# Regenerator/dpf-nets

Hardware: AMD Instinct MI355X
Metric: points/sec through 14-layer flow + Chamfer, B=32 N=2048 (higher is better)
Workload: dtype f16x3 MFMA operands, fp32 accumulate/points; 1 GPU; configs[1]: airplane autoencoder shapes, B=32 N=2048 per GPU: 14 coupling layers (first 14 of LocalCondRNVPDecoder(n_flows=5)), direct/eval-BN, + nn_distance both directions + CD reduction; clouds_per_gpu=32, points_per_cloud=2048, hidden=64, latent=128, global_clouds=32, per_layer_lists=False, launch=hipGraph replay, 10 step(s) per graph, steps_in_flight=1, settle_steps=400, parallelism=clouds sharded, no collective, sclk_mhz=2239, chamfer_impl=auto (matrix-core filtered exact search at this size)

## Files before the change

### dpf_nets_amd/csrc/chamfer_mfma.hip

```cpp
#include <hip/hip_runtime.h>
#include <limits.h>
#include <stdint.h>
#include <stdlib.h>

#include "dpf_hip.h"
#include "lds_attr.h"
#include "zero_fill.h"
#include "nn_refscan.h"

#pragma clang fp contract(off)

namespace {

typedef __bf16 bf16x8 __attribute__((ext_vector_type(8)));
typedef float f32x16 __attribute__((ext_vector_type(16)));
typedef uint32_t u32x4 __attribute__((ext_vector_type(4)));

constexpr int CT = dispatch::NNM_CT;
constexpr int PROW = 100;
constexpr int SCH = 32;
constexpr int WCAP = SCH * 64 / 8;
constexpr int NNM_PTS = CT * 1024, NNM_LISTS = NNM_PTS + CT * PROW * 4;
__host__ __device__ constexpr int nnm_lds_bytes(int qw) { return NNM_LISTS + qw * SCH * 64 + qw * WCAP * 2; }

__device__ __forceinline__ uint32_t f2u(float x) { return __builtin_bit_cast(uint32_t, x); }
__device__ __forceinline__ float u2f(uint32_t x) { return __builtin_bit_cast(float, x); }
__device__ __forceinline__ uint32_t bf16_rne(float x) {
    const uint32_t u = f2u(x);
    return (u + 0x7FFFu + ((u >> 16) & 1u)) >> 16;
}
__device__ __forceinline__ void split2(float x, uint32_t &hi, uint32_t &lo) {
    const uint32_t h = f2u(x) & 0xFFFF0000u;
    hi = h >> 16;
    lo = bf16_rne(x - u2f(h));
}

__host__ __device__ inline int tiles_of(int n) { return (n + 31) / 32; }

__device__ __forceinline__ void cand_coord(float c, uint32_t &w0, uint32_t &w1) {
    uint32_t hi, lo;
    split2(c, hi, lo);
    w0 = hi | (hi << 16);
    w1 = lo | (lo << 16);
}
__device__ __forceinline__ void cand_fragment(float x, float y, float z, bool live, uint4 &h0, uint4 &h1) {
    cand_coord(x, h0.x, h0.y);
    cand_coord(y, h0.z, h0.w);
    cand_coord(z, h1.x, h1.y);
    const float w = (x * x + y * y) + z * z;
    const float ww = live ? w : 3.0e38f;
    const uint32_t wh = f2u(ww) & 0xFFFF0000u;
    const float r1 = ww - u2f(wh);
    const uint32_t wm = f2u(r1) & 0xFFFF0000u;
    const float r2 = r1 - u2f(wm);
    h1.z = (wh >> 16) | (live ? wm : 0u);
    h1.w = live ? bf16_rne(r2) : 0u;
}
__device__ __forceinline__ uint4 query_fragment(float x, float y, float z, int h) {
    uint32_t ah, al, bh, bl;
    split2(-2.0f * (h ? z : x), ah, al);
    split2(-2.0f * y, bh, bl);
    uint4 o;
    o.x = ah | (al << 16); o.y = o.x;
    o.z = h ? 0x3F803F80u : (bh | (bl << 16));
    o.w = h ? 0x00003F80u : o.z;
    return o;
}

struct MDir {
    const float *q, *c;
    float *dist;
    int *idx;
    int nq, nc;
    long qstride, cstride;
};
struct MArgs {
    MDir d[2]; int pn2; float *part; unsigned *ticket; float *cd;
#ifdef DPF_PROFILE
    unsigned long long *prof;
#endif
};

__device__ __forceinline__ f32x16 mfma(uint4 a, uint4 b) {
    const f32x16 z = {0.f, 0.f, 0.f, 0.f, 0.f, 0.f, 0.f, 0.f, 0.f, 0.f, 0.f, 0.f, 0.f, 0.f, 0.f, 0.f};
    return __builtin_amdgcn_mfma_f32_32x32x16_bf16(__builtin_bit_cast(bf16x8, a), __builtin_bit_cast(bf16x8, b), z, 0, 0, 0);
}
__device__ __forceinline__ float tile_min(const f32x16 &s) {
    float m = fminf(fminf(s[0], s[1]), s[2]);
    m = fminf(fminf(m, s[3]), s[4]);   m = fminf(fminf(m, s[5]), s[6]);
    m = fminf(fminf(m, s[7]), s[8]);   m = fminf(fminf(m, s[9]), s[10]);
    m = fminf(fminf(m, s[11]), s[12]); m = fminf(fminf(m, s[13]), s[14]);
    return fminf(fminf(m, s[15]), s[0]);
}
__device__ __forceinline__ float dist3(float cx, float cy, float cz, float qx, float qy, float qz) {
    const float dx = cx - qx, dy = cy - qy, dz = cz - qz;
    return (dx * dx + dy * dy) + dz * dz;
}
template <class P>
__device__ __forceinline__ void exact_tile(P cp, int nc, int t, int tl, int h, float qx, float qy, float qz,
                                           float &best, int &bidx) {
    float d[16];
#pragma unroll
    for (int g = 0; g < 4; ++g) {
        const float *row = cp + (size_t)tl * PROW + 8 * g + 4 * h;
        const float4 vx = *(const float4 *)row, vy = *(const float4 *)(row + 32), vz = *(const float4 *)(row + 64);
        d[4 * g + 0] = dist3(vx.x, vy.x, vz.x, qx, qy, qz); d[4 * g + 1] = dist3(vx.y, vy.y, vz.y, qx, qy, qz);
        d[4 * g + 2] = dist3(vx.z, vy.z, vz.z, qx, qy, qz); d[4 * g + 3] = dist3(vx.w, vy.w, vz.w, qx, qy, qz);
    }
    float m = fminf(fminf(d[0], d[1]), d[2]);
#pragma unroll
    for (int r = 3; r < 15; r += 2) m = fminf(fminf(m, d[r]), d[r + 1]);
    m = fminf(m, d[15]);
    if (m <= best) {
        int kmin = INT_MAX;
#pragma unroll
        for (int r = 15; r >= 0; --r) {
            const int k = t * 32 + 8 * (r >> 2) + 4 * h + (r & 3);
            kmin = (d[r] == m && k < nc) ? k : kmin;
        }
        const bool better = kmin != INT_MAX && (m < best || kmin < bidx);
        best = better ? m : best;
        bidx = better ? kmin : bidx;
    }
}

template <class P>
__device__ __forceinline__ void exact_tile_mk(P cp, int nc, int t, int tl, int h, float qx, float qy, float qz, float &m, int &kmin) {
    float d[16];
#pragma unroll
    for (int g = 0; g < 4; ++g) {
        const float *row = cp + (size_t)tl * PROW + 8 * g + 4 * h;
        const float4 vx = *(const float4 *)row, vy = *(const float4 *)(row + 32), vz = *(const float4 *)(row + 64);
        d[4 * g + 0] = dist3(vx.x, vy.x, vz.x, qx, qy, qz); d[4 * g + 1] = dist3(vx.y, vy.y, vz.y, qx, qy, qz);
        d[4 * g + 2] = dist3(vx.z, vy.z, vz.z, qx, qy, qz); d[4 * g + 3] = dist3(vx.w, vy.w, vz.w, qx, qy, qz);
    }
    m = fminf(fminf(d[0], d[1]), d[2]);
#pragma unroll
    for (int r = 3; r < 15; r += 2) m = fminf(fminf(m, d[r]), d[r + 1]);
    m = fminf(m, d[15]);
    int rmin = 16;
#pragma unroll
    for (int r = 15; r >= 0; --r) rmin = d[r] == m ? r : rmin;
    const int k = t * 32 + 8 * (rmin >> 2) + 4 * h + (rmin & 3);
    kmin = (rmin < 16 && k < nc) ? k : INT_MAX;
}

template <int CTRL, int ROW_MASK = 0xF>
__device__ __forceinline__ unsigned dpp_or0(unsigned v) {
    return (unsigned)__builtin_amdgcn_update_dpp(0, (int)v, CTRL, ROW_MASK, 0xF, true);
}
__device__ __forceinline__ unsigned wave_scan_add(unsigned v) {
    v += dpp_or0<0x111>(v); v += dpp_or0<0x112>(v); v += dpp_or0<0x114>(v); v += dpp_or0<0x118>(v);
    v += dpp_or0<0x142, 0xA>(v);
    v += dpp_or0<0x143, 0xC>(v);
    return v;
}
__device__ __forceinline__ unsigned wave_max_u32(unsigned v) {
    v = max(v, dpp_or0<0x111>(v)); v = max(v, dpp_or0<0x112>(v)); v = max(v, dpp_or0<0x114>(v)); v = max(v, dpp_or0<0x118>(v));
    v = max(v, dpp_or0<0x142, 0xA>(v));
    v = max(v, dpp_or0<0x143, 0xC>(v));
    return (unsigned)__builtin_amdgcn_readlane((int)v, 63);
}

#ifdef DPF_PROFILE
#define DPF_T(i) { __builtin_amdgcn_sched_barrier(0); \
    if (prof_at != nullptr) { const unsigned long long t_ = __builtin_amdgcn_s_memtime(); if ((threadIdx.x & 63) == 0) prof_at[i] = t_; } \
    __builtin_amdgcn_sched_barrier(0); }
#else
#define DPF_T(i)
#endif

typedef __attribute__((address_space(3))) void lds_void;
typedef __attribute__((address_space(1))) const void glb_void;

template <int QW>
__global__ __launch_bounds__(QW * 64) void nnm_kernel(MArgs args) {
    extern __shared__ __attribute__((aligned(16))) uint8_t lds[];
    unsigned char *qtile = (unsigned char *)(lds + NNM_LISTS);
    __shared__ float s_r2[QW], s_sum[QW];
    const bool pairwise = args.pn2 > 0;
    const int dir = pairwise ? (int)(blockIdx.z & 1) : (int)blockIdx.z;
    const MDir A = args.d[dir];
    const int pi = pairwise ? (int)(blockIdx.z >> 1) : 0, pj = (int)blockIdx.y;
    const int bi = pairwise ? 0 : (int)blockIdx.y;
    const int nq = A.nq, nc = A.nc;
    const bool sums = args.part != nullptr;
    const size_t part_at = pairwise ? (((size_t)pi * args.pn2 + pj) * 2 + dir) * gridDim.x + blockIdx.x
                                    : ((size_t)bi * 2 + dir) * gridDim.x + blockIdx.x;
    const size_t unit = pairwise ? (size_t)pi * args.pn2 + pj : (size_t)bi;
    auto publish = [&](float t) {
        if (args.ticket == nullptr) { args.part[part_at] = t; return; }
        __hip_atomic_store(&args.part[part_at], t, __ATOMIC_RELAXED, __HIP_MEMORY_SCOPE_AGENT);
        asm volatile("s_waitcnt vmcnt(0)" ::: "memory");
        const unsigned nwg2 = 2u * gridDim.x;
        const unsigned old = __hip_atomic_fetch_add(&args.ticket[unit], 1u, __ATOMIC_RELAXED, __HIP_MEMORY_SCOPE_AGENT);
        if (old == nwg2 - 1) {
            const float *p = args.part + unit * nwg2;
            float s1 = 0.f, s2 = 0.f;
            for (unsigned x0 = 0; x0 < gridDim.x; x0 += 4) {
                float v1[4], v2[4];
#pragma unroll
                for (unsigned u = 0; u < 4; ++u) {
                    const unsigned x = min(x0 + u, gridDim.x - 1);
                    v1[u] = __hip_atomic_load(&p[x], __ATOMIC_RELAXED, __HIP_MEMORY_SCOPE_AGENT);
                    v2[u] = __hip_atomic_load(&p[gridDim.x + x], __ATOMIC_RELAXED, __HIP_MEMORY_SCOPE_AGENT);
                }
#pragma unroll
                for (unsigned u = 0; u < 4; ++u)
                    if (x0 + u < gridDim.x) { s1 += v1[u]; s2 += v2[u]; }
            }
            args.cd[unit] = s1 / (float)args.d[0].nq + s2 / (float)args.d[1].nq;
            __hip_atomic_store(&args.ticket[unit], 0u, __ATOMIC_RELAXED, __HIP_MEMORY_SCOPE_AGENT);
        }
    };
    if ((int)blockIdx.x * QW * 32 >= nq) {
        if (sums && threadIdx.x == 0) publish(0.f);
        return;
    }
    const int tid = threadIdx.x, lane = tid & 63, h = lane >> 5;
    const int wave = __builtin_amdgcn_readfirstlane(tid >> 6);
#ifdef DPF_PROFILE
    unsigned long long *prof_at = nullptr;
    if (args.prof != nullptr && blockIdx.y < 2 && blockIdx.z == 0 && gridDim.x <= 4)
        prof_at = args.prof + ((size_t)(blockIdx.y * gridDim.x + blockIdx.x) * QW + wave) * 16;
#endif
    DPF_T(0)
    const int qt = blockIdx.x * QW + wave;
    const int nqt = tiles_of(nq), nct = tiles_of(nc);
    const bool wave_live = qt < nqt;
    const size_t qcloud = pairwise ? (size_t)(dir == 0 ? pi : pj) * A.qstride : (size_t)bi * A.qstride;
    const size_t ccloud = pairwise ? (size_t)(dir == 0 ? pj : pi) * A.cstride : (size_t)bi * A.cstride;
    const float *__restrict__ cpts = A.c + ccloud;
    const int j = qt * 32 + (lane & 31);
    const float *qsrc = A.q + qcloud + (size_t)min(j, nq - 1) * 3;
    const float qx = qsrc[0], qy = qsrc[1], qz = qsrc[2];
    constexpr int KPT = CT * 32 / (QW * 64);
    const int npass = (nct + CT - 1) / CT;
    float px[KPT], py[KPT], pz[KPT];
#pragma unroll
    for (int k = 0; k < KPT; ++k) {
        const int p = tid + k * QW * 64;
        px[k] = 0.f; py[k] = 0.f; pz[k] = 0.f;
        if (p < nc) { const float *src = cpts + (size_t)p * 3; px[k] = src[0]; py[k] = src[1]; pz[k] = src[2]; }
    }
    float mux, muy, muz;
    {
        const float *src = cpts + (size_t)min(lane, nc - 1) * 3;
        mux = src[0]; muy = src[1]; muz = src[2];
        for (int d = 32; d > 0; d >>= 1) { mux += __shfl_xor(mux, d); muy += __shfl_xor(muy, d); muz += __shfl_xor(muz, d); }
        mux *= 0.015625f; muy *= 0.015625f; muz *= 0.015625f;
    }
    const float qcx = qx - mux, qcy = qy - muy, qcz = qz - muz;
    const uint4 bq = query_fragment(qcx, qcy, qcz, h);
    const float INF_ = __builtin_inff();
    float r2 = j < nq ? (qcx * qcx + qcy * qcy) + qcz * qcz : 0.f;
    r2 = nn_not_finite(r2) ? INF_ : r2;
    DPF_T(1)
    if (nct > CT)
        for (int p = tid; p < nc; p += QW * 64) {
            const float *src = cpts + (size_t)p * 3;
            const float x = src[0] - mux, y = src[1] - muy, z = src[2] - muz;
            const float cn = (x * x + y * y) + z * z;
            r2 = nn_not_finite(cn) ? INF_ : fmaxf(r2, cn);
        }

    uint4 *sfrag = (uint4 *)lds;
    float *spts = (float *)(lds + NNM_PTS);
    auto put = [&](int pl, bool live, float x, float y, float z) {
        const int t = pl >> 5, i = pl & 31;
        uint4 f0, f1;
        const float cx = live ? x - mux : 0.f, cy = live ? y - muy : 0.f, cz = live ? z - muz : 0.f;
        cand_fragment(cx, cy, cz, live, f0, f1);
        sfrag[t * 64 + i] = f0;
        sfrag[t * 64 + 32 + i] = f1;
        spts[t * PROW + i] = live ? x : 3.0e38f; spts[t * PROW + 32 + i] = live ? y : 3.0e38f; spts[t * PROW + 64 + i] = live ? z : 3.0e38f;
        return (cx * cx + cy * cy) + cz * cz;
    };
    {
        const int tn = min(CT, nct);
        int tidp = tid;
        asm volatile("" : "+v"(tidp));
#pragma unroll
        for (int k = 0; k < KPT; ++k) {
            const int pl = tidp + k * QW * 64;
            if ((pl >> 5) < tn) {
                const float cn = put(pl, pl < nc, px[k], py[k], pz[k]);
                r2 = nn_not_finite(cn) ? INF_ : fmaxf(r2, cn);
            }
        }
    }
    DPF_T(2)
    const float r2w = u2f(wave_max_u32(f2u(r2)));
    if (lane == 0) s_r2[wave] = r2w;
    __syncthreads();
    float tau;
    bool slow;
    {
        float m = s_r2[0];
#pragma unroll
        for (int w = 1; w < QW; ++w) m = fmaxf(m, s_r2[w]);
        tau = m * 2.44140625e-4f;
        slow = nn_not_finite(m);
    }
    DPF_T(3)

    unsigned short *wl = (unsigned short *)(lds + NNM_LISTS + QW * SCH * 64) + (size_t)wave * WCAP;
    uint2 *res = (uint2 *)(qtile + (size_t)wave * SCH * 64);
    float smin = __builtin_inff();
    float best = __builtin_inff();
    int bidx = INT_MAX;
    for (int pass = 0; pass < (slow ? 0 : npass); ++pass) {
        const int t0 = pass * CT, tn = min(CT, nct - t0);
        if (pass > 0) {
            __syncthreads();
            int tidp = tid;
            asm volatile("" : "+v"(tidp));
#pragma unroll
            for (int k = 0; k < KPT; ++k) {
                const int pl = tidp + k * QW * 64, p = t0 * 32 + pl;
                if ((pl >> 5) < tn) {
                    const bool live = p < nc;
                    float x = 0.f, y = 0.f, z = 0.f;
                    if (live) { const float *src = cpts + (size_t)p * 3; x = src[0]; y = src[1]; z = src[2]; }
                    put(pl, live, x, y, z);
                }
            }
            __syncthreads();
        }
        if (wave_live) {
            for (int c0 = 0; c0 < tn; c0 += SCH) {
                const int cn = min(SCH, tn - c0);
                float mt[SCH];
                if (cn == SCH) {
                    const uint4 *fr = sfrag + c0 * 64 + lane;
                    if constexpr (QW < 16) {
                        uint4 fa = fr[0], fb = fr[64];
                        f32x16 a = mfma(fa, bq);
                        fa = fr[2 * 64];
#pragma unroll
                        for (int u = 0; u < SCH; u += 2) {
                            const f32x16 b = mfma(fb, bq);
                            if (u + 3 < SCH) fb = fr[(u + 3) * 64];
                            __builtin_amdgcn_sched_barrier(0);
                            mt[u] = tile_min(a);
                            __builtin_amdgcn_sched_barrier(0);
                            if (u + 2 < SCH) {
                                a = mfma(fa, bq);
                                if (u + 4 < SCH) fa = fr[(u + 4) * 64];
                            }
                            __builtin_amdgcn_sched_barrier(0);
                            mt[u + 1] = tile_min(b);
                            __builtin_amdgcn_sched_barrier(0);
                        }
                    } else {
                        f32x16 a = mfma(fr[0], bq);
#pragma unroll
                        for (int u = 0; u < SCH; u += 2) {
                            const f32x16 b = mfma(fr[(u + 1) * 64], bq);
                            __builtin_amdgcn_sched_barrier(0);
                            mt[u] = tile_min(a);
                            __builtin_amdgcn_sched_barrier(0);
                            if (u + 2 < SCH) a = mfma(fr[(u + 2) * 64], bq);
                            __builtin_amdgcn_sched_barrier(0);
                            mt[u + 1] = tile_min(b);
                            __builtin_amdgcn_sched_barrier(0);
                        }
                    }
                } else {
                    auto frag = [&](int u) { return sfrag[(c0 + min(u, cn - 1)) * 64 + lane]; };
                    f32x16 a = mfma(frag(0), bq);
#pragma unroll
                    for (int u = 0; u < SCH; u += 2) {
                        const f32x16 b = mfma(frag(u + 1), bq);
                        __builtin_amdgcn_sched_barrier(0);
                        mt[u] = tile_min(a);
                        __builtin_amdgcn_sched_barrier(0);
                        if (u + 2 < SCH) a = mfma(frag(u + 2), bq);
                        __builtin_amdgcn_sched_barrier(0);
                        mt[u + 1] = tile_min(b);
                        __builtin_amdgcn_sched_barrier(0);
                    }
                }
                DPF_T(4 + 5 * (c0 / SCH))
                float cm = fminf(fminf(mt[0], mt[1]), mt[2]);
#pragma unroll
                for (int u = 3; u + 1 < SCH; u += 2) cm = fminf(fminf(cm, mt[u]), mt[u + 1]);
                cm = fminf(cm, mt[SCH - 1]);
                smin = fminf(smin, cm);
                const float thr = fminf(smin, __shfl_xor(smin, 32)) + tau;
                unsigned smask = 0;
                static_assert(SCH == 32, "the mask is built sixteen tiles at a time, twice");
#define NNM_MK(n) "v_cmp_le_f32 vcc, %" #n ", %17\n\tv_addc_co_u32 %0, vcc, %0, %0, vcc\n\t"
#pragma unroll
                for (int u = 0; u < SCH; u += 16)
                    asm(NNM_MK(1) NNM_MK(2) NNM_MK(3) NNM_MK(4) NNM_MK(5) NNM_MK(6) NNM_MK(7) NNM_MK(8)
                        NNM_MK(9) NNM_MK(10) NNM_MK(11) NNM_MK(12) NNM_MK(13) NNM_MK(14) NNM_MK(15) NNM_MK(16)
                        : "+v"(smask)
                        : "v"(mt[u]), "v"(mt[u + 1]), "v"(mt[u + 2]), "v"(mt[u + 3]), "v"(mt[u + 4]), "v"(mt[u + 5]), "v"(mt[u + 6]),
                          "v"(mt[u + 7]), "v"(mt[u + 8]), "v"(mt[u + 9]), "v"(mt[u + 10]), "v"(mt[u + 11]), "v"(mt[u + 12]),
                          "v"(mt[u + 13]), "v"(mt[u + 14]), "v"(mt[u + 15]), "v"(thr)
                        : "vcc");
#undef NNM_MK
                if (cn < SCH) smask &= ~0u << (SCH - cn);
                const int nsurv = __builtin_popcount(smask);
                DPF_T(5 + 5 * (c0 / SCH))
                int off = (int)wave_scan_add((unsigned)nsurv);
                const int W = __builtin_amdgcn_readlane(off, 63);
                off -= nsurv;
                if (W <= WCAP) {
                    {
                        unsigned mk = smask;
                        for (int e = 0; __builtin_amdgcn_ballot_w64(mk != 0) != 0; ++e) {
                            if (mk != 0) wl[off + e] = (unsigned short)((lane << 8) | (SCH - 1 - __builtin_ctz(mk)));
                            mk &= mk - 1;
                        }
                    }
                    DPF_T(6 + 5 * (c0 / SCH))
                    __builtin_amdgcn_fence(__ATOMIC_RELEASE, "wavefront");
                    __builtin_amdgcn_wave_barrier();
                    for (int i0 = 0; i0 < W; i0 += 64) {
                        const int i = i0 + lane;
                        const unsigned item = wl[min(i, W - 1)];
                        const int sl = (int)(item >> 8), tl = c0 + (int)(item & 255u);
                        const float sx = __shfl(qx, sl), sy = __shfl(qy, sl), sz = __shfl(qz, sl);
                        float m; int k;
                        exact_tile_mk(spts, nc, t0 + tl, tl, sl >> 5, sx, sy, sz, m, k);
                        if (i < W) res[i] = make_uint2(__float_as_uint(m), (unsigned)k);
                    }
                    __builtin_amdgcn_fence(__ATOMIC_RELEASE, "wavefront");
                    __builtin_amdgcn_wave_barrier();
                    DPF_T(7 + 5 * (c0 / SCH))
                    for (int e = 0; __builtin_amdgcn_ballot_w64(e < nsurv) != 0; ++e) {
                        if (e < nsurv) {
                            const uint2 r = res[off + e];
                            const float m = __uint_as_float(r.x);
                            const int k = (int)r.y;
                            const bool better = k != INT_MAX && (m < best || (m == best && k < bidx));
                            best = better ? m : best;
                            bidx = better ? k : bidx;
                        }
                    }
                    __builtin_amdgcn_fence(__ATOMIC_RELEASE, "wavefront");
                    __builtin_amdgcn_wave_barrier();
                    DPF_T(8 + 5 * (c0 / SCH))
                } else {
                    const int smax = (int)wave_max_u32((unsigned)nsurv);
                    unsigned mk = smask;
                    for (int e = 0; e < smax; ++e) {
                        const bool take = mk != 0;
                        const int tl = c0 + (take ? SCH - 1 - __builtin_ctz(mk) : 0);
                        mk &= mk - 1;
                        float b2 = best; int i2 = bidx;
                        exact_tile(spts, nc, t0 + tl, tl, h, qx, qy, qz, b2, i2);
                        if (take) { best = b2; bidx = i2; }
                    }
                }
            }
        }
    }
    if (slow && wave_live)
        nn_reference_scan(cpts, nc, qx, qy, qz, best, bidx);
    if (!wave_live && !sums) return;
    const float od = __shfl_xor(best, 32);
    const int oi = __shfl_xor(bidx, 32);
    if (od < best || (od == best && oi < bidx)) { best = od; bidx = oi; }
    int tid_out = threadIdx.x;
    asm volatile("" : "+v"(tid_out));
    const int j_out = (blockIdx.x * QW + (tid_out >> 6)) * 32 + (tid_out & 31);
    if (!pairwise) {
        if (wave_live && h == 0 && j_out < nq) {
            A.dist[(size_t)bi * nq + j_out] = best;
            A.idx[(size_t)bi * nq + j_out] = bidx;
        }
        if (!sums) return;
    }
    DPF_T(14)
    float sum = (wave_live && h == 0 && j_out < nq) ? best : 0.f;
    for (int d = 16; d > 0; d >>= 1) sum += __shfl_xor(sum, d);
    if (lane == 0) s_sum[wave] = sum;
    __syncthreads();
    if (tid == 0) {
        float t = s_sum[0];
#pragma unroll
        for (int w = 1; w < QW; ++w) t += s_sum[w];
        publish(t);
    }
    DPF_T(15)
}

__global__ __launch_bounds__(64) void nnm_surrogate_kernel(const float *__restrict__ q, int nq, const float *__restrict__ c, int nc,
                                                           float *__restrict__ s, float *__restrict__ out3) {
    __shared__ uint4 frag[64];
    const int lane = threadIdx.x, h = lane >> 5, i = lane & 31, qt = blockIdx.x, ct = blockIdx.y;
    float mux, muy, muz;
    {
        const float *src = c + (size_t)min(lane, nc - 1) * 3;
        mux = src[0]; muy = src[1]; muz = src[2];
        for (int d = 32; d > 0; d >>= 1) { mux += __shfl_xor(mux, d); muy += __shfl_xor(muy, d); muz += __shfl_xor(muz, d); }
        mux *= 0.015625f; muy *= 0.015625f; muz *= 0.015625f;
    }
    const int j = qt * 32 + i, p = ct * 32 + i;
    const float *qsrc = q + (size_t)min(j, nq - 1) * 3;
    const uint4 bq = query_fragment(qsrc[0] - mux, qsrc[1] - muy, qsrc[2] - muz, h);
    if (h == 0) {
        const bool live = p < nc;
        const float *src = c + (size_t)min(p, nc - 1) * 3;
        uint4 f0, f1;
        cand_fragment(live ? src[0] - mux : 0.f, live ? src[1] - muy : 0.f, live ? src[2] - muz : 0.f, live, f0, f1);
        frag[i] = f0; frag[32 + i] = f1;
    }
    __syncthreads();
    const f32x16 a = mfma(frag[lane], bq);
#pragma unroll
    for (int r = 0; r < 16; ++r) {
        const int k = ct * 32 + 8 * (r >> 2) + 4 * h + (r & 3);
        if (j < nq && k < nc) s[(size_t)j * nc + k] = a[r];
    }
    if (qt == 0 && ct == 0) {
        float r2 = 0.f;
#pragma clang loop vectorize(disable) interleave(disable)
        for (int t = lane; t < nq + nc; t += 64) {
            const float *src = t < nq ? q + (size_t)t * 3 : c + (size_t)(t - nq) * 3;
            const float x = src[0] - mux, y = src[1] - muy, z = src[2] - muz;
            r2 = fmaxf(r2, (x * x + y * y) + z * z);
        }
        for (int d = 32; d > 0; d >>= 1) r2 = fmaxf(r2, __shfl_xor(r2, d));
        if (lane == 0) { out3[0] = mux; out3[1] = muy; out3[2] = muz; out3[3] = r2; }
    }
}

}

extern "C" int dpf_debug_nn_surrogate(int nq, const float *q, int nc, const float *c, float *s, float *out4, dpf_stream_t stream) {
    if (nq <= 0 || nc <= 0 || !q || !c || !s || !out4) return DPF_EINVAL;
    hipLaunchKernelGGL(nnm_surrogate_kernel, dim3(tiles_of(nq), tiles_of(nc)), dim3(64), 0, (hipStream_t)stream, q, nq, c, nc, s, out4);
    return (int)hipGetLastError();
}

extern "C" size_t dpf_nndistance_mfma_workspace_bytes(int b, int n, int m) {
    (void)b; (void)n; (void)m;
    return 0;
}

#ifdef DPF_PROFILE
static unsigned long long *g_nnm_prof = nullptr;
extern "C" void dpf_debug_set_nnm_prof(void *p) { g_nnm_prof = (unsigned long long *)p; }
#endif

template <int QW>
static int launch_nnm_qw(const MArgs &ma, int b, int nmax, hipStream_t s) {
    const int lds = nnm_lds_bytes(QW);
    static LdsLimit limit;
    if (hipError_t e = limit.ensure((const void *)nnm_kernel<QW>, lds); e != hipSuccess) return (int)e;
    hipLaunchKernelGGL(nnm_kernel<QW>, dim3((nmax + QW * 32 - 1) / (QW * 32), b, 2), dim3(QW * 64), lds, s, ma);
    return (int)hipGetLastError();
}

static int launch_nnm(int b, int n, const float *xyz, long xyz_stride, int m, const float *xyz2, long xyz2_stride, float *result,
                      int *result_i, float *result2, int *result2_i, const dispatch::Switches &sw, hipStream_t s,
                      float *part = nullptr, bool force16 = false, unsigned *ticket = nullptr, float *cd = nullptr) {
    MArgs ma;
    ma.pn2 = 0; ma.part = part; ma.ticket = ticket; ma.cd = cd;
#ifdef DPF_PROFILE
    ma.prof = g_nnm_prof;
#endif
    ma.d[0] = MDir{xyz, xyz2, result, result_i, n, m, xyz_stride, xyz2_stride};
    ma.d[1] = MDir{xyz2, xyz, result2, result2_i, m, n, xyz2_stride, xyz_stride};
    const int nmax = n > m ? n : m;
    switch (dispatch::nnm_qw(b, n, m, force16, sw)) {
    case 16: return launch_nnm_qw<16>(ma, b, nmax, s);
    case 8: return launch_nnm_qw<8>(ma, b, nmax, s);
    default: return launch_nnm_qw<4>(ma, b, nmax, s);
    }
}

static int nn_auto(int b, int n, const float *xyz, long xyz_stride, int m, const float *xyz2, long xyz2_stride, float *result,
                   int *result_i, float *result2, int *result2_i, const dispatch::Switches &sw, hipStream_t s) {
    if (xyz && xyz2 && result && result_i && result2 && result2_i && xyz_stride >= 0 && xyz2_stride >= 0 && dispatch::nnm_pays(b, n, m, sw))
        return launch_nnm(b, n, xyz, xyz_stride, m, xyz2, xyz2_stride, result, result_i, result2, result2_i, sw, s);
    return nn_scan_strided(b, n, xyz, xyz_stride, m, xyz2, xyz2_stride, result, result_i, result2, result2_i, sw, s);
}

extern "C" int dpf_nndistance_mfma(int b, int n, const float *xyz, int m, const float *xyz2, float *result,
                                   int *result_i, float *result2, int *result2_i, void *workspace,
                                   size_t workspace_bytes, dpf_stream_t stream) {
    (void)workspace; (void)workspace_bytes;
    if (b < 0 || n <= 0 || m <= 0) return DPF_EINVAL;
    if (b == 0) return 0;
    if (!xyz || !xyz2 || !result || !result_i || !result2 || !result2_i) return DPF_EINVAL;
    const dispatch::Switches sw = dispatch::snapshot();
    if (b > 65535 || n > 65535 * 32 || m > 65535 * 32 || (n < 32 && m < 32))
        return nn_scan_strided(b, n, xyz, (long)n * 3, m, xyz2, (long)m * 3, result, result_i, result2, result2_i, sw, (hipStream_t)stream);
    return launch_nnm(b, n, xyz, (long)n * 3, m, xyz2, (long)m * 3, result, result_i, result2, result2_i, sw, (hipStream_t)stream);
}

extern "C" int dpf_nndistance_auto(int b, int n, const float *xyz, int m, const float *xyz2, float *result, int *result_i,
                                   float *result2, int *result2_i, dpf_stream_t stream) {
    return nn_auto(b, n, xyz, (long)n * 3, m, xyz2, (long)m * 3, result, result_i, result2, result2_i, dispatch::snapshot(),
                   (hipStream_t)stream);
}

extern "C" int dpf_nndistance_strided_auto(int b, int n, const float *xyz, long xyz_stride, int m, const float *xyz2,
                                           long xyz2_stride, float *result, int *result_i, float *result2, int *result2_i,
                                           dpf_stream_t stream) {
    return nn_auto(b, n, xyz, xyz_stride, m, xyz2, xyz2_stride, result, result_i, result2, result2_i, dispatch::snapshot(),
                   (hipStream_t)stream);
}

extern "C" size_t dpf_pairwise_cd_workspace_bytes(int n1, int n2, int n, int m) {
    const int nmax = n > m ? n : m, per = dispatch::pairwise_qw(nmax) * 32;
    return (size_t)n1 * n2 * (2 * ((nmax + per - 1) / per) + 1) * sizeof(float);
}
extern "C" int dpf_pairwise_cd(int n1, int n2, int n, int m, const float *clouds1, const float *clouds2, float *cds,
                               void *workspace, size_t workspace_bytes, dpf_stream_t stream) {
    if (n1 < 0 || n2 < 0 || n <= 0 || m <= 0) return DPF_EINVAL;
    if (n1 == 0 || n2 == 0) return 0;
    if (!clouds1 || !clouds2 || !cds || !workspace) return DPF_EINVAL;
    if (workspace_bytes < dpf_pairwise_cd_workspace_bytes(n1, n2, n, m)) return DPF_EINVAL;
    if (n2 > 65535 || n1 > 32767 || n < 32 || m < 32 || n > 65535 * 32 || m > 65535 * 32) return DPF_ENOSUP;
    MArgs ma;
    ma.d[0] = MDir{clouds1, clouds2, nullptr, nullptr, n, m, (long)n * 3, (long)m * 3};
    ma.d[1] = MDir{clouds2, clouds1, nullptr, nullptr, m, n, (long)m * 3, (long)n * 3};
    const int nmax = n > m ? n : m, qw = dispatch::pairwise_qw(nmax), nwg = (nmax + qw * 32 - 1) / (qw * 32);
    const long npairs = (long)n1 * n2;
    hipStream_t s = (hipStream_t)stream;
    ma.pn2 = n2; ma.ticket = (unsigned *)workspace; ma.part = (float *)workspace + npairs; ma.cd = cds;
#ifdef DPF_PROFILE
    ma.prof = nullptr;
#endif
    if (hipError_t e = dpf_zero_async(workspace, (size_t)npairs * sizeof(unsigned), s); e != hipSuccess) return (int)e;
    if (qw == 16) {
        const int lds = nnm_lds_bytes(16);
        static LdsLimit limit;
        if (hipError_t e = limit.ensure((const void *)nnm_kernel<16>, lds); e != hipSuccess) return (int)e;
        hipLaunchKernelGGL(nnm_kernel<16>, dim3(nwg, n2, 2 * n1), dim3(16 * 64), lds, s, ma);
    } else {
        const int lds = nnm_lds_bytes(8);
        static LdsLimit limit;
        if (hipError_t e = limit.ensure((const void *)nnm_kernel<8>, lds); e != hipSuccess) return (int)e;
        hipLaunchKernelGGL(nnm_kernel<8>, dim3(nwg, n2, 2 * n1), dim3(8 * 64), lds, s, ma);
    }
    return (int)hipGetLastError();
}

extern "C" size_t dpf_nndistance_cd_workspace_bytes(int b, int n, int m) {
    const int nmax = n > m ? n : m;
    return (size_t)(b > 0 ? b : 0) * (2 * ((nmax + 63) / 64) + 1) * sizeof(float) + 16;
}
extern "C" int dpf_nndistance_cd(int b, int n, const float *xyz, int m, const float *xyz2, float *result, int *result_i,
                                 float *result2, int *result2_i, float *cd, void *workspace, size_t workspace_bytes,
                                 int tickets_are_zero, dpf_stream_t stream) {
    if (b < 0 || n <= 0 || m <= 0) return DPF_EINVAL;
    if (b == 0) return 0;
    if (!xyz || !xyz2 || !result || !result_i || !result2 || !result2_i || !cd) return DPF_EINVAL;
    hipStream_t s = (hipStream_t)stream;
    const dispatch::Switches sw = dispatch::snapshot();
    const bool ws_ok = workspace && workspace_bytes >= dpf_nndistance_cd_workspace_bytes(b, n, m), pays = dispatch::nnm_pays(b, n, m, sw);
    if (ws_ok && pays) {
        if (!tickets_are_zero)
            if (hipError_t e = dpf_zero_async(workspace, (size_t)b * sizeof(unsigned), s); e != hipSuccess) return (int)e;
        return launch_nnm(b, n, xyz, (long)n * 3, m, xyz2, (long)m * 3, result, result_i, result2, result2_i, sw, s,
                          (float *)workspace + b, false, (unsigned *)workspace, cd);
    }
    if (ws_ok) {
        const int rc = nn_small_cd(b, n, xyz, m, xyz2, result, result_i, result2, result2_i, cd, workspace, tickets_are_zero, sw, s);
        if (rc != DPF_ENOSUP) return rc;
    }
    if (int rc = nn_auto(b, n, xyz, (long)n * 3, m, xyz2, (long)m * 3, result, result_i, result2, result2_i, sw, s)) return rc;
    return dpf_chamfer_reduce(b, n, m, result, result2, cd, stream);
}
```

Before: 967.4 million points/s.

## Defer first chunk's survivors and refine both chunks in one merged work list

Instead of building a work list and running the exact-refine pass after every 32-tile chunk, the first chunk's survivor mask is held in registers. It is re-filtered against the tighter threshold known after the second chunk, and then both chunks' survivors go through a single scan, list build and exact pass. This is meant to cut the number of partially filled 64-lane refine rounds and drop more first-chunk candidates. The cost is extra register pressure, plus a static_assert that a pass holds at most two chunks.

```diff
diff --git a/dpf_nets_amd/csrc/chamfer_mfma.hip b/dpf_nets_amd/csrc/chamfer_mfma.hip
--- a/dpf_nets_amd/csrc/chamfer_mfma.hip
+++ b/dpf_nets_amd/csrc/chamfer_mfma.hip
@@ -328,6 +328,10 @@
             __syncthreads();
         }
         if (wave_live) {
+            static_assert(CT <= 2 * SCH, "one chunk waits in registers: a pass is at most two chunks");
+            static_assert(CT <= 256, "a work item names its tile of the pass in eight bits");
+            unsigned dmask = 0, smask = 0;
+            float dcm = 0.f, thr = 0.f;
             for (int c0 = 0; c0 < tn; c0 += SCH) {
                 const int cn = min(SCH, tn - c0);
                 float mt[SCH];
@@ -381,14 +385,14 @@
                         __builtin_amdgcn_sched_barrier(0);
                     }
                 }
-                DPF_T(4 + 5 * (c0 / SCH))
+                DPF_T(4 + 2 * (c0 / SCH))
                 float cm = fminf(fminf(mt[0], mt[1]), mt[2]);
 #pragma unroll
                 for (int u = 3; u + 1 < SCH; u += 2) cm = fminf(fminf(cm, mt[u]), mt[u + 1]);
                 cm = fminf(cm, mt[SCH - 1]);
                 smin = fminf(smin, cm);
-                const float thr = fminf(smin, __shfl_xor(smin, 32)) + tau;
-                unsigned smask = 0;
+                thr = fminf(smin, __shfl_xor(smin, 32)) + tau;
+                smask = 0;
                 static_assert(SCH == 32, "the mask is built sixteen tiles at a time, twice");
 #define NNM_MK(n) "v_cmp_le_f32 vcc, %" #n ", %17\n\tv_addc_co_u32 %0, vcc, %0, %0, vcc\n\t"
 #pragma unroll
@@ -402,58 +406,74 @@
                         : "vcc");
 #undef NNM_MK
                 if (cn < SCH) smask &= ~0u << (SCH - cn);
-                const int nsurv = __builtin_popcount(smask);
-                DPF_T(5 + 5 * (c0 / SCH))
-                int off = (int)wave_scan_add((unsigned)nsurv);
-                const int W = __builtin_amdgcn_readlane(off, 63);
-                off -= nsurv;
-                if (W <= WCAP) {
-                    {
-                        unsigned mk = smask;
-                        for (int e = 0; __builtin_amdgcn_ballot_w64(mk != 0) != 0; ++e) {
-                            if (mk != 0) wl[off + e] = (unsigned short)((lane << 8) | (SCH - 1 - __builtin_ctz(mk)));
-                            mk &= mk - 1;
-                        }
+                DPF_T(5 + 2 * (c0 / SCH))
+                if (c0 + SCH < tn) { dmask = smask; dcm = cm; }
+            }
+#ifdef DPF_PROFILE
+            const unsigned dmask_all = dmask;
+#endif
+            dmask = dcm <= thr ? dmask : 0u;
+            const int lb = (tn > SCH ? SCH : 0) + SCH - 1;
+            const int n0 = __builtin_popcount(dmask), nsurv = n0 + __builtin_popcount(smask);
+            int off = (int)wave_scan_add((unsigned)nsurv);
+            const int W = __builtin_amdgcn_readlane(off, 63);
+            off -= nsurv;
+#ifdef DPF_PROFILE
+            if (prof_at != nullptr) {
+                const int w0 = __builtin_amdgcn_readlane((int)wave_scan_add((unsigned)__builtin_popcount(dmask_all)), 63);
+                const int w1 = __builtin_amdgcn_readlane((int)wave_scan_add((unsigned)__builtin_popcount(smask)), 63);
+                if (lane == 0) { prof_at[11] = (W + 63) / 64; prof_at[12] = (w0 + 63) / 64 + (w1 + 63) / 64; prof_at[13] = W; }
+            }
+#endif
+            if (W <= WCAP) {
+                {
+                    unsigned mk0 = dmask, mk1 = smask;
+                    for (int e = 0; __builtin_amdgcn_ballot_w64((mk0 | mk1) != 0) != 0; ++e) {
+                        if (mk0 != 0) wl[off + e] = (unsigned short)((lane << 8) | (SCH - 1 - __builtin_ctz(mk0)));
+                        if (mk1 != 0) wl[off + n0 + e] = (unsigned short)((lane << 8) | (lb - __builtin_ctz(mk1)));
+                        mk0 &= mk0 - 1;
+                        mk1 &= mk1 - 1;
                     }
-                    DPF_T(6 + 5 * (c0 / SCH))
-                    __builtin_amdgcn_fence(__ATOMIC_RELEASE, "wavefront");
-                    __builtin_amdgcn_wave_barrier();
-                    for (int i0 = 0; i0 < W; i0 += 64) {
-                        const int i = i0 + lane;
-                        const unsigned item = wl[min(i, W - 1)];
-                        const int sl = (int)(item >> 8), tl = c0 + (int)(item & 255u);
-                        const float sx = __shfl(qx, sl), sy = __shfl(qy, sl), sz = __shfl(qz, sl);
-                        float m; int k;
-                        exact_tile_mk(spts, nc, t0 + tl, tl, sl >> 5, sx, sy, sz, m, k);
-                        if (i < W) res[i] = make_uint2(__float_as_uint(m), (unsigned)k);
+                }
+                DPF_T(8)
+                __builtin_amdgcn_fence(__ATOMIC_RELEASE, "wavefront");
+                __builtin_amdgcn_wave_barrier();
+                for (int i0 = 0; i0 < W; i0 += 64) {
+                    const int i = i0 + lane;
+                    const unsigned item = wl[min(i, W - 1)];
+                    const int sl = (int)(item >> 8), tl = (int)(item & 255u);
+                    const float sx = __shfl(qx, sl), sy = __shfl(qy, sl), sz = __shfl(qz, sl);
+                    float m; int k;
+                    exact_tile_mk(spts, nc, t0 + tl, tl, sl >> 5, sx, sy, sz, m, k);
+                    if (i < W) res[i] = make_uint2(__float_as_uint(m), (unsigned)k);
+                }
+                __builtin_amdgcn_fence(__ATOMIC_RELEASE, "wavefront");
+                __builtin_amdgcn_wave_barrier();
+                DPF_T(9)
+                for (int e = 0; __builtin_amdgcn_ballot_w64(e < nsurv) != 0; ++e) {
+                    if (e < nsurv) {
+                        const uint2 r = res[off + e];
+                        const float m = __uint_as_float(r.x);
+                        const int k = (int)r.y;
+                        const bool better = k != INT_MAX && (m < best || (m == best && k < bidx));
+                        best = better ? m : best;
+                        bidx = better ? k : bidx;
                     }
-                    __builtin_amdgcn_fence(__ATOMIC_RELEASE, "wavefront");
-                    __builtin_amdgcn_wave_barrier();
-                    DPF_T(7 + 5 * (c0 / SCH))
-                    for (int e = 0; __builtin_amdgcn_ballot_w64(e < nsurv) != 0; ++e) {
-                        if (e < nsurv) {
-                            const uint2 r = res[off + e];
-                            const float m = __uint_as_float(r.x);
-                            const int k = (int)r.y;
-                            const bool better = k != INT_MAX && (m < best || (m == best && k < bidx));
-                            best = better ? m : best;
-                            bidx = better ? k : bidx;
-                        }
-                    }
-                    __builtin_amdgcn_fence(__ATOMIC_RELEASE, "wavefront");
-                    __builtin_amdgcn_wave_barrier();
-                    DPF_T(8 + 5 * (c0 / SCH))
-                } else {
-                    const int smax = (int)wave_max_u32((unsigned)nsurv);
-                    unsigned mk = smask;
-                    for (int e = 0; e < smax; ++e) {
-                        const bool take = mk != 0;
-                        const int tl = c0 + (take ? SCH - 1 - __builtin_ctz(mk) : 0);
-                        mk &= mk - 1;
-                        float b2 = best; int i2 = bidx;
-                        exact_tile(spts, nc, t0 + tl, tl, h, qx, qy, qz, b2, i2);
-                        if (take) { best = b2; bidx = i2; }
-                    }
+                }
+                __builtin_amdgcn_fence(__ATOMIC_RELEASE, "wavefront");
+                __builtin_amdgcn_wave_barrier();
+                DPF_T(10)
+            } else {
+                const int smax = (int)wave_max_u32((unsigned)nsurv);
+                unsigned mk0 = dmask, mk1 = smask;
+                for (int e = 0; e < smax; ++e) {
+                    const bool first = mk0 != 0, take = (mk0 | mk1) != 0;
+                    const int tl = first ? SCH - 1 - __builtin_ctz(mk0) : mk1 != 0 ? lb - __builtin_ctz(mk1) : 0;
+                    mk1 = first ? mk1 : mk1 & (mk1 - 1);
+                    mk0 &= mk0 - 1;
+                    float b2 = best; int i2 = bidx;
+                    exact_tile(spts, nc, t0 + tl, tl, h, qx, qy, qz, b2, i2);
+                    if (take) { best = b2; bidx = i2; }
                 }
             }
         }
```

Result: faster. 978.6 million points/s, median of 6 (+1.1%).
